# ajaayc/Probability-of-Collision-for-Safe-Planning

Hardware: AMD Instinct MI355X
Metric: particle-waypoint evals/s (GMM+collision) (higher is better)
Workload: dtype f64

## Files before the change

### probability-of-collision-for-safe-planning_amd/csrc/pocs_ctx.hpp

```cpp
#pragma once
#include <hip/hip_runtime.h>

#include <math.h>
#include <stdarg.h>
#include <stdio.h>
#include <stdlib.h>
#include <string.h>

#include <algorithm>
#include <string>
#include <vector>

#include "../../include/pocs.h"
#include "pocs_kernels.h"

#define POCS_HIDDEN __attribute__((visibility("hidden")))

namespace pocs_rt POCS_HIDDEN {

struct DevBuf {
  void* p = nullptr;
  size_t cap = 0;
};

// ... 98 lines not shown
    bool valid = false;
    uint64_t seed = 0, run_index = 0;
    int R = 0;
    unsigned long long epoch = 0;
    std::vector<double> image, chain0, mu0, cov0;
    std::vector<int> slot_plan;
  } ahead;

  pocs_rt::DevBuf d_env, d_sensor, d_hdr, d_chain, d_state, d_param, d_moments, d_partial;
  pocs_rt::DevBuf d_sx, d_sy, d_st, d_flags, d_px, d_py, d_pt, d_hits, d_total, d_ticket, d_tables;
  pocs_rt::DevBuf d_runplan;
  pocs_rt::DevBuf d_surv;
  pocs_rt::DevBuf d_tparent;
  pocs_rt::DevBuf d_world, d_kept, d_keptidx, d_reach;
  pocs_rt::DevBuf d_obsct;
  void* xchg_own = nullptr;
  void* xchg_peer[POCS_XCHG_MAX_WORLD] = {nullptr, nullptr, nullptr, nullptr, nullptr, nullptr, nullptr, nullptr};
  int xchg_world = 0, xchg_rank = -1;
  bool xchg_connected = false;
  unsigned long long xchg_calls = 0;
  double* ext_moments = nullptr;
  long long ext_moments_len = 0;
  void* h_pin = nullptr;
  size_t h_pin_cap = 0;
  void* h_copy = nullptr;
  bool env_dirty = true, sensor_dirty = true;

  hipGraphExec_t graph_gmm = nullptr, graph_mc = nullptr;
  const void* graph_baked[3] = {nullptr, nullptr, nullptr};
  std::string graph_gmm_key, graph_mc_key;

  std::vector<hipEvent_t> events;
  double prof_ms = 0.0;
  long long prof_launches = 0;

  pocs_rt::Results res;
  int last_gmm_adv = -1;
  bool gmm_open = false;
};

namespace pocs_rt POCS_HIDDEN {

inline int fail(pocs_ctx* c, int code, const char* fmt, ...) {
  char buf[512];
  va_list ap;
  va_start(ap, fmt);
  vsnprintf(buf, sizeof buf, fmt, ap);
  va_end(ap);
  if (c) c->err = buf;
  return code;
}

#define HIPCHK(c, call)                                                                   \
  do {                                                                                    \
    hipError_t e_ = (call);                                                               \
    if (e_ != hipSuccess)                                                                 \
      return fail((c), POCS_E_DEVICE, "%s failed: %s (%s:%d)", #call, hipGetErrorString(e_), \
                  __FILE__, __LINE__);                                                    \
  } while (0)

inline void drop_graphs(pocs_ctx* c) {
  if (c->graph_gmm) { hipGraphExecDestroy(c->graph_gmm); c->graph_gmm = nullptr; }
  if (c->graph_mc) { hipGraphExecDestroy(c->graph_mc); c->graph_mc = nullptr; }
  c->graph_gmm_key.clear();
  c->graph_mc_key.clear();
}

inline int ensure(pocs_ctx* c, DevBuf& b, size_t bytes) {
  if (bytes == 0) bytes = 16;
  if (b.cap >= bytes) return POCS_OK;
  if (b.p) {
    HIPCHK(c, hipStreamSynchronize(c->stream));
    drop_graphs(c);
    HIPCHK(c, hipFree(b.p)); b.p = nullptr; b.cap = 0;
  }
  HIPCHK(c, hipMalloc(&b.p, bytes));
  b.cap = bytes;
  return POCS_OK;
}

inline void ra_drop(pocs_ctx* c) {
  if (c->ra_have > 0) c->run_index = c->res.batch_base + (uint64_t)c->res.view + 1;
  c->ra_have = 0;
}
inline void touch(pocs_ctx* c) { ra_drop(c); c->epoch++; }

inline void reset_results(pocs_ctx* c) {
  Results& r = c->res;
// ... 4 lines not shown
  r.plan_slot[0].clear(); r.plan_slot[1].clear(); r.plan_E.clear();
  r.mc_wp.clear(); r.mc_wp_W = 0; r.plan_E_mc.clear();
  r.tree_last = 0; r.tree_sel = 0; r.tree_mc_half = 0;
  r.tree_probs.clear(); r.tree_eval.clear(); r.tree_F.clear(); r.tree_C.clear();
  r.oc_kind = 0; r.oc_M = 0; r.oc_W = 0;
}

inline int world_boxes(const pocs_ctx* c) { return (int)(c->boxes.size() / 5 / (size_t)c->world_S); }
inline const pocs_env_dev* world_at(const pocs_ctx* c, int w) {
  return (const pocs_env_dev*)c->d_env.p + (w < 0 ? 0 : w < c->world_S ? w : c->world_S - 1);
}

static_assert(POCS_MAX_WORLD_RECORDS == POCS_MAX_WORLD_BOXES, "pocs_kernels.h restates the public limit");
inline bool large_world(const pocs_ctx* c) { return !c->world.empty(); }
inline int large_boxes(const pocs_ctx* c) { return (int)(c->world.size() / 5); }

inline double* moments_dev(pocs_ctx* c) { return c->ext_moments ? c->ext_moments : (double*)c->d_moments.p; }
inline long long sample_stride_of(long long count) { return count > 0 ? ((count + 1) & ~1LL) : 2; }
inline uint64_t seed_of_run(const pocs_ctx* c, uint64_t run) { return c->seed + 0x9E3779B97F4A7C15ull * run; }

struct PlanView { const double* traj; const double* odom; int W; };
PlanView plan_view(const pocs_ctx* c, int p);
void compute_chain(pocs_ctx* c, uint64_t seed, const PlanView& pv);
struct PinLayout { size_t chain, state0, runplan, moments, total, end; };
PinLayout pin_layout(const pocs_ctx* c);
int ensure_pin(pocs_ctx* c);
std::vector<int> plan_layout(const pocs_ctx* c, int G);
std::vector<int> slot_lengths(const pocs_ctx* c, const std::vector<int>& slot_plan);
int live_runs(const std::vector<int>& Ws, int lo, int hi, int w);
uint64_t plan_run(const pocs_ctx* c, int p);
void prefetch_next_batch(pocs_ctx* c, int groups);
int stage_and_upload_runs(pocs_ctx* c, int groups, int kind);

int upload_tables(pocs_ctx* c);
int upload_world(pocs_ctx* c);
void fill_gmm_world(const pocs_ctx* c, pocs_gmm_launch* a, int w);
size_t obs_count_words(const pocs_ctx* c);
size_t sync_xwait_offset(const pocs_ctx* c);
void gmm_select_view(pocs_ctx* c, int v);
void tree_select_gmm(pocs_ctx* c, int n);
int run_gmm_full(pocs_ctx* c, double* probability);
int run_mc_local(pocs_ctx* c);

}
```

### probability-of-collision-for-safe-planning_amd/csrc/pocs_host.hip

```cpp
#include <chrono>

#include "pocs_ctx.hpp"

namespace pocs_rt POCS_HIDDEN {

int grid_blocks(long long count, int block, int bpc) {
  long long nb = (count + block - 1) / block;
  if (nb < 1) nb = 1;
  if (nb > 256LL * bpc) nb = 256LL * bpc;
  if (nb > POCS_MAX_BLOCKS) nb = POCS_MAX_BLOCKS;
  return (int)nb;
}
#define POCS_FULL_GRID_FROM_RUNS 4
struct GmmGeometry { long long chunks; int vs_shift; int upb; int blocks; };
GmmGeometry gmm_geometry(long long count, int runs, int K, int groups = 1) {
  const int tb = POCS_GMM_BLOCK_OF(K);
  const long long npairs = (count + 1) / 2;
  GmmGeometry g;
  g.chunks = (npairs + tb - 1) / tb;
  if (g.chunks < 1) g.chunks = 1;
  g.vs_shift = 0;
  while ((2LL << g.vs_shift) <= g.chunks && (2 << g.vs_shift) <= POCS_GMM_MAX_VS) ++g.vs_shift;
  if (runs < 1) runs = 1;
  const long long units = (long long)runs << g.vs_shift;
// ... 112 lines not shown

size_t obs_count_words(const pocs_ctx* c) { return (size_t)c->batch * (size_t)(c->W > 0 ? c->W : 1) * POCS_MAX_OBSTACLES; }
int ensure_obs_counts(pocs_ctx* c) {
  return c->opt_obs_counts ? ensure(c, c->d_obsct, obs_count_words(c) * sizeof(unsigned long long)) : POCS_OK;
}
int enqueue_obs_counts_reset(pocs_ctx* c) {
  if (!c->opt_obs_counts) return POCS_OK;
  HIPCHK(c, pocs_launch_zero_counts((unsigned long long*)c->d_obsct.p, obs_count_words(c), c->stream));
  return POCS_OK;
}
void note_obs_counts(pocs_ctx* c, int kind) {
  c->res.oc_kind = c->opt_obs_counts ? kind : 0;
  c->res.oc_M = world_boxes(c);
  c->res.oc_W = c->W > 0 ? c->W : 1;
}

size_t sync_stop_offset(const pocs_ctx*) { return 4; }
size_t sync_ticket_offset(const pocs_ctx* c) { return 4 + (risk_active(c) ? (((size_t)c->batch + 3) & ~(size_t)3) : 0); }
size_t sync_xwait_offset(const pocs_ctx* c) { return sync_ticket_offset(c) + (size_t)c->batch * (size_t)(c->W > 0 ? c->W : 1); }
size_t sync_words(const pocs_ctx* c) {
  const size_t n = sync_xwait_offset(c) + (size_t)c->batch * (size_t)(c->W > 0 ? c->W : 1);
  return (n + 3) & ~(size_t)3;
}

int gmm_prepare(pocs_ctx* c) {
  if (int r = check_common(c)) return r;
  if (c->K < 1) return fail(c, POCS_E_STATE, "setNumGaussians missing");
  if (c->num_gmm < 1) return fail(c, POCS_E_STATE, "setNumGMMSamples missing");
  long long first, count;
  if (int r = gmm_shard(c, &first, &count)) return r;
  if (int r = upload_static(c)) return r;
  const size_t W = (size_t)c->W, K = (size_t)c->K, R = (size_t)c->batch;
  const GmmGeometry geo = gmm_geometry(count, c->batch, c->K);
  if (int r = ensure(c, c->d_hdr, R * sizeof(pocs_run_header))) return r;
  if (int r = ensure(c, c->d_chain, R * (W > 1 ? W - 1 : 1) * POCS_CHAIN_STRIDE * sizeof(double))) return r;
  if (int r = ensure(c, c->d_state, R * W * K * POCS_STATE_STRIDE * sizeof(double))) return r;
  if (int r = ensure(c, c->d_param, R * W * K * POCS_PARAM_STRIDE * sizeof(double))) return r;
  if (!c->ext_moments)
    if (int r = ensure(c, c->d_moments, W * R * K * POCS_NMOM * sizeof(double))) return r;
  if (c->ext_moments && c->ext_moments_len < (long long)(W * R * K * POCS_NMOM))
    return fail(c, POCS_E_BUFFER, "bound moments buffer too small");
  if (int r = ensure(c, c->d_partial, 2 * ((c->tree.n && R > 256 ? (size_t)256 : R) << geo.vs_shift) * K * POCS_NMOM * sizeof(double))) return r;
  if (int r = ensure(c, c->d_ticket, sync_words(c) * sizeof(unsigned))) return r;
  if (c->plans.n)
    if (int r = ensure(c, c->d_runplan, R * 4 * sizeof(double))) return r;
  if (risk_active(c))
    if (int r = ensure(c, c->d_surv, R * sizeof(double))) return r;
  if (c->tree.n)
    if (int r = upload_tree(c)) return r;
  if (int r = ensure_obs_counts(c)) return r;
  if (large_world(c)) {
    if (int r = ensure(c, c->d_kept, R * POCS_MAX_OBSTACLES * POCS_OBS_STRIDE * sizeof(double))) return r;
    if (int r = ensure(c, c->d_keptidx, R * POCS_MAX_OBSTACLES * sizeof(int))) return r;
    if (int r = ensure(c, c->d_reach, R * W * sizeof(int))) return r;
  }
  if (c->opt_store && !c->tree.n) {
    const size_t n = R * (size_t)sample_stride_of(count);
    if (int r = ensure(c, c->d_sx, n * sizeof(double))) return r;
    if (int r = ensure(c, c->d_sy, n * sizeof(double))) return r;
    if (int r = ensure(c, c->d_st, n * sizeof(double))) return r;
    if (int r = ensure(c, c->d_flags, n * sizeof(int16_t))) return r;
  }
  return ensure_pin(c);
}

int gmm_groups(const pocs_ctx* c) {
  if (c->ext_moments) return 1;
  if (c->tree.n) return 1;
  int g = (int)c->opt_groups;
  if (g == 0) {
    const double count = (double)(c->shard_first >= 0 ? c->shard_count : c->num_gmm);
    g = (c->batch >= 8 && (double)c->batch * count >= 1.2e6) ? 2 : 1;
  }
  if (g > c->batch) g = c->batch;
  return g < 1 ? 1 : g;
}

int gmm_upload_run(pocs_ctx* c) {
  if (int r = stage_and_upload_runs(c, gmm_groups(c), 0)) return r;
  const PinLayout pl = pin_layout(c);
  double* pin = (double*)c->h_pin;
  const int W = c->W, R = c->batch;
  const size_t row = (size_t)c->K * POCS_STATE_STRIDE * sizeof(double);
  HIPCHK(c, hipMemcpy2DAsync(c->d_state.p, (size_t)W * row, pin + pl.state0, row, row, (size_t)(c->tree.n ? 1 : R),
                             hipMemcpyHostToDevice, c->stream));
  return POCS_OK;
}

bool whole_call_exchanges(const pocs_ctx* c) { return c->xchg_connected && c->shard_first >= 0 && !c->ext_moments; }

void fill_gmm_world(const pocs_ctx* c, pocs_gmm_launch* a, int w) {
  a->env = world_at(c, w);
  a->tables = (const pocs_tables*)c->d_tables.p;
  a->fp = c->fp; a->M = world_boxes(c);
  a->fp_rr = sqrt(c->fp.hx * c->fp.hx + c->fp.hy * c->fp.hy); a->fp_phi = atan2(c->fp.hy, c->fp.hx);
  if (large_world(c)) {
    a->world = (const double*)c->d_world.p; a->world_M = large_boxes(c);
    a->kept = (double*)c->d_kept.p; a->kept_idx = (int*)c->d_keptidx.p; a->reach = (int*)c->d_reach.p;
  }
}

void fill_gmm_launch(pocs_ctx* c, pocs_gmm_launch* a, long long first, long long count, int w,
// ... 125 lines not shown
          continue;
        }
      }
      if (int r = enqueue_step(c, first, count, w, true, exchange, (prof && g == 0) ? w : -1, st, lo, cnt, G, lone, adv, risk)) return r;
    }
  if (lone) {
    pocs_gmm_launch a;
    fill_gmm_launch(c, &a, first, count, W - 1, 0, 1, 1);
    set_lone(c, &a, W - 1);
    HIPCHK(c, pocs_launch_gmm_close(c->K, a, c->stream));
  }
  for (int g = 1; g < G; ++g) {
    HIPCHK(c, hipEventRecord(c->ev_join[g - 1], c->side_stream[g - 1]));
    HIPCHK(c, hipStreamWaitEvent(c->stream, c->ev_join[g - 1], 0));
  }
  if (prof) HIPCHK(c, hipEventRecord(c->ev_seq[1], c->stream));
  return POCS_OK;
}
int enqueue_gmm_results(pocs_ctx* c) {
  const int W = c->W;
  const PinLayout pl = pin_layout(c);
  HIPCHK(c, hipMemcpyAsync((double*)c->h_pin + pl.moments, moments_dev(c),
                           (size_t)W * c->batch * c->K * POCS_NMOM * sizeof(double), hipMemcpyDeviceToHost, c->stream));
  static_assert(POCS_SYNC_ABORT == 1, "the stop words follow the give-up word and two pad words");
  HIPCHK(c, hipMemcpyAsync((double*)c->h_pin + pl.total + c->batch + 1, (unsigned*)c->d_ticket.p + POCS_SYNC_ABORT,
                           (risk_active(c) ? 3 + (size_t)c->batch : 1) * sizeof(unsigned), hipMemcpyDeviceToHost, c->stream));
  if (large_world(c)) {
    c->reach.assign((size_t)c->batch * (size_t)c->W, 0);
    HIPCHK(c, hipMemcpyAsync(c->reach.data(), c->d_reach.p, c->reach.size() * sizeof(int), hipMemcpyDeviceToHost, c->stream));
  }
  return POCS_OK;
}

int gmm_read_reach(pocs_ctx* c) {
  const int R = c->batch, W = c->W;
  const bool plans = c->plans.n && !c->res.plan_slot[0].empty();
  const std::vector<int> by_slot = c->reach;
  c->reach_R = R; c->reach_W = W;
  c->reach_len.assign((size_t)R, W);
  int bad_w = -1, bad_n = 0, bad_r = 0;
  for (int r = 0; r < R; ++r) {
    const int slot = plans ? c->res.plan_slot[0][(size_t)r] : r;
    if (plans) c->reach_len[(size_t)r] = c->plans.W[(size_t)r];
    for (int w = 0; w < W; ++w) {
      const int n = by_slot[(size_t)slot * W + w];
      c->reach[(size_t)r * W + w] = n;
      if (n > POCS_MAX_OBSTACLES && (bad_w < 0 || w < bad_w)) { bad_w = w; bad_n = n; bad_r = r; }
    }
  }
  if (bad_w >= 0)
    return fail(c, POCS_E_STATE, "large world: %d boxes are in reach of run %d at waypoint %d, more than the %d a run may meet at one waypoint; results discarded",
                bad_n, bad_r, bad_w, POCS_MAX_OBSTACLES);
  return POCS_OK;
}

double waypoint_probability(const double* row, int K, long long n) {
  double coll = 0.0;
  for (int k = 0; k < K; ++k) coll += row[(size_t)k * POCS_NMOM + 1];
  return coll / (1.0 * (double)n);
}
// ... 137 lines not shown
  HIPCHK(c, e);
  e = hipGraphInstantiate(&exec, g, nullptr, nullptr, 0);
  hipGraphDestroy(g);
  HIPCHK(c, e);
  have = key;
  return POCS_OK;
}

int run_gmm_full(pocs_ctx* c, double* probability) {
  if (!probability) return fail(c, POCS_E_ARG, "null output");
#if defined(POCS_TUNING) && defined(POCS_CALL_TIMES)
  const auto t_in = std::chrono::steady_clock::now();
  auto lap = [&](const char* what) { fprintf(stderr, "[call] %s +%.1f us\n", what,
      std::chrono::duration<double, std::micro>(std::chrono::steady_clock::now() - t_in).count()); };
#else
  auto lap = [](const char*) {};
#endif
  c->res.oc_kind = 0;
  c->reach.clear(); c->reach_len.clear(); c->reach_R = 0; c->reach_W = 0;
  if (int r = gmm_prepare(c)) return r;
  long long first, count;
  if (int r = gmm_shard(c, &first, &count)) return r;
  lap("prepared");
  if (whole_call_exchanges(c)) {
    if (c->batch > POCS_XCHG_MAX_RUNS) return fail(c, POCS_E_ARG, "exchange: at most %d runs per call", POCS_XCHG_MAX_RUNS);
    c->xchg_calls += 1;
  }
  if (int r = gmm_upload_run(c)) return r;
  lap("upload enqueued");
  const bool prof = c->opt_profile == 1 && !c->tree.n, span = c->opt_profile == 2 && c->opt_graph;
  if (int r = prof_begin(c, gmm_hot_launches(c))) return r;
#if defined(POCS_TUNING) && defined(POCS_GRAPH_WITH_COPIES)
  const bool copies_in_graph = c->opt_graph && !prof;
#else
  const bool copies_in_graph = false;
#endif
  if (!copies_in_graph) if (int r = enqueue_ticket_reset(c)) return r;
  if (c->opt_graph && c->opt_profile != 1) {
    if (int r = ensure_graph(c, c->graph_gmm, c->graph_gmm_key, config_key(c, first, count, "gmm"), [&] {
          int r = copies_in_graph ? enqueue_ticket_reset(c) : POCS_OK;
          if (!r) r = enqueue_gmm_all(c, first, count, false);
          if (!r && copies_in_graph) r = enqueue_gmm_results(c);
          if (copies_in_graph) {
            c->graph_baked[0] = c->d_ticket.p; c->graph_baked[1] = c->h_pin; c->graph_baked[2] = moments_dev(c);
          }
          return r;
        })) return r;
    if (copies_in_graph && (c->graph_baked[0] != c->d_ticket.p || c->graph_baked[1] != c->h_pin || c->graph_baked[2] != moments_dev(c)))
      return fail(c, POCS_E_STATE, "a pointer baked into the graph's memset / memcpy nodes changed between capture and replay");
    if (span) HIPCHK(c, hipEventRecord(c->ev_seq[0], c->stream));
    HIPCHK(c, hipGraphLaunch(c->graph_gmm, c->stream));
    if (span) HIPCHK(c, hipEventRecord(c->ev_seq[1], c->stream));
  } else {
    if (int r = enqueue_gmm_all(c, first, count, prof)) return r;
  }
  if (!copies_in_graph) if (int r = enqueue_gmm_results(c)) return r;
  lap("launched");
  prefetch_next_batch(c, gmm_groups(c));
  lap("next batch prepared");
  HIPCHK(c, hipStreamSynchronize(c->stream));
  lap("synchronised");
  if (prof) if (int r = prof_collect(c, gmm_hot_launches(c))) return r;
  if (prof || span) {
    float ms = 0.f;
    HIPCHK(c, hipEventElapsedTime(&ms, c->ev_seq[0], c->ev_seq[1]));
    c->seq_ms = ms; c->seq_groups = gmm_groups(c);
    if (span) { c->prof_ms = ms; c->prof_launches = (long long)gmm_hot_launches(c); }
  }
  {
    const PinLayout pl = pin_layout(c);
    unsigned gave_up = 0;
    memcpy(&gave_up, (double*)c->h_pin + pl.total + c->batch + 1, sizeof gave_up);
    if (gave_up) return fail(c, POCS_E_DEVICE, "a bounded wait expired on the device (code %u); results discarded", gave_up);
    const unsigned* stop = risk_active(c) ? (const unsigned*)((double*)c->h_pin + pl.total + c->batch + 1) + 3 : nullptr;
    if (large_world(c)) if (int r = gmm_read_reach(c)) { reset_results(c); return r; }
    if (int r = gmm_combine(c, (double*)c->h_pin + pl.moments, probability, stop)) { reset_results(c); return r; }
  }
  note_obs_counts(c, 1);
  c->res.last_gmm_count = count;
  c->res.last_gmm_wp = c->W - 1;
  lap("combined");
  return POCS_OK;
}

int mc_shard(pocs_ctx* c, long long* first, long long* count) {
  *first = c->shard_first >= 0 ? c->shard_first : 0;
  *count = c->shard_first >= 0 ? c->shard_count : c->num_particles;
  if (*first < 0 || *count < 0 || *first + *count > c->num_particles)
    return fail(c, POCS_E_ARG, "shard [%lld,+%lld) outside numParticles=%lld", *first, *count, c->num_particles);
  return POCS_OK;
}

bool mc_stop_active(const pocs_ctx* c) { return c->opt_mc_rb && risk_active(c) && !c->tree.n; }
bool mc_counts_active(const pocs_ctx* c) { return c->opt_mc_wp || c->opt_obs_counts || mc_stop_active(c); }
bool mc_fused_form(const pocs_ctx* c) { return c->opt_fused && !mc_stop_active(c); }
size_t mc_total_words(const pocs_ctx* c) {
  const size_t R = (size_t)c->batch, W = (size_t)c->W;
// ... 367 lines not shown
  a.xchg.world = c->xchg_world; a.xchg.rank = c->xchg_rank;
  a.xchg.epoch = (c->xchg_calls << 20) | (unsigned long long)(w + 1);
  a.xchg.parity = (int)((c->xchg_calls * (unsigned long long)c->W + (unsigned long long)w) & 1ull);
  const int slot = c->opt_profile == 1 ? w : -1;
  if (slot >= 0) HIPCHK(c, hipEventRecord(c->events[2 * slot], c->stream));
  HIPCHK(c, pocs_launch_gmm_step(c->K, a, c->stream));
  if (slot >= 0) HIPCHK(c, hipEventRecord(c->events[2 * slot + 1], c->stream));
  c->res.last_gmm_wp = w;
  c->res.last_gmm_count = count;
  if (w + 1 < c->W) c->last_gmm_adv = w + 1;
  return POCS_OK;
}

int pocs_gmm_end(pocs_ctx* c, double* probability) {
  if (!c) return POCS_E_ARG;
  if (!c->gmm_open) return fail(c, POCS_E_ORDER, "pocs_gmm_end before pocs_gmm_begin");
  if (c->res.last_gmm_wp != c->W - 1) return fail(c, POCS_E_ORDER, "pocs_gmm_end after %d of %d waypoints", c->res.last_gmm_wp + 1, c->W);
  if (!probability) return fail(c, POCS_E_ARG, "null output");
  const PinLayout pl = pin_layout(c);
  if (int r = enqueue_gmm_results(c)) return r;
  prefetch_next_batch(c, gmm_groups(c));
  HIPCHK(c, hipStreamSynchronize(c->stream));
  unsigned gave_up = 0;
  memcpy(&gave_up, (double*)c->h_pin + pl.total + c->batch + 1, sizeof gave_up);
  if (gave_up) { c->gmm_open = false; return fail(c, POCS_E_DEVICE, "a bounded wait expired on the device (code %u: 4 = a peer's moments never arrived); results discarded", gave_up); }
  if (int r = prof_collect(c, (size_t)c->W)) return r;
  (void)gmm_combine(c, (double*)c->h_pin + pl.moments, probability);
  note_obs_counts(c, 1);
  c->gmm_open = false;
  return POCS_OK;
}

}
```

### probability-of-collision-for-safe-planning_amd/csrc/pocs_kernels.h

```cpp
#pragma once
#include <hip/hip_runtime.h>
#include <stdint.h>
#include "pocs_collide.h"
#include "pocs_model.h"
#include "pocs_world.h"

#define POCS_BLOCK 256
#define POCS_GMM_BLOCK_OF(K) 512
#define POCS_GMM_BLOCKS_PER_CU 2
#define POCS_NUM_CUS 256
#define POCS_MAX_BLOCKS 2048
#define POCS_GMM_MAX_VS 256
static_assert(POCS_GMM_BLOCK_OF(3) == 512 && POCS_GMM_MAX_VS == 256, "summation tree (numerics v7 and later): 512-pair chunks, 256 virtual slices");
#define POCS_LONE_PRE 3
#define POCS_GMM_SUB 32
#define POCS_UNIT_SUMS 10
#define POCS_FLUSH_ROWS 5
#define POCS_FLUSH_PITCH 66
#define POCS_CHAIN_Z 10
#define POCS_CHAIN_STRIDE 48
static_assert(POCS_CHAIN_Z + POCS_MAX_LANDMARKS <= POCS_CHAIN_STRIDE, "chain record too small");

struct pocs_env_dev {
  pocs_footprint fp;
// ... 91 lines not shown
  double mu0[3];
  double L0[6];
  const double* run_plan;
  int step;
  int nruns;
  int nontemporal;
  int wp_mode;
  unsigned long long* wp_counts;
  unsigned* wp_stop;
  long long wp_n;
  double wp_bound;
  const int* tree_parent;
  const double* tree_sx; const double* tree_sy; const double* tree_sth;
  const uint32_t* tree_shits;
  int tree_lo, tree_dst_lo, tree_src_lo, tree_pad;
  int env_steps;
  int env_pad;
  unsigned long long* obs_counts;
  const double* world;
  int world_M;
  int world_pad;
};


hipError_t pocs_launch_gmm_step(int K, const pocs_gmm_launch& a, hipStream_t s);
hipError_t pocs_launch_world_cull(int K, const pocs_gmm_launch& a, hipStream_t s);
hipError_t pocs_launch_gmm_advance(int K, const pocs_gmm_launch& a, hipStream_t s);
hipError_t pocs_launch_gmm_tree_advance(int K, const pocs_gmm_launch& a, hipStream_t s);
hipError_t pocs_launch_gmm_tree_step(int K, const pocs_gmm_launch& a, hipStream_t s);
hipError_t pocs_launch_gmm_close(int K, const pocs_gmm_launch& a, hipStream_t s);
hipError_t pocs_launch_gmm_exchange(int K, const pocs_gmm_launch& a, const pocs_xchg_dev& x, hipStream_t s);
hipError_t pocs_launch_zero_counts(unsigned long long* p, size_t words, hipStream_t s);
hipError_t pocs_launch_copy(const void* src, void* dst, long long bytes, hipStream_t s);
hipError_t pocs_launch_fill(void* dst, long long bytes, hipStream_t s);
hipError_t pocs_launch_probe_math(const pocs_tables* tables, int n, const uint32_t* wr, const uint32_t* wa, const double* x, double* out, hipStream_t s);
hipError_t pocs_launch_probe_collide(int K, const pocs_gmm_launch& a, int n, const double* x, const double* y, const double* th,
                                     int* flags, int* nkeep, double* kept, hipStream_t s);
hipError_t pocs_launch_mc_init(int nblk, const pocs_mc_launch& a, hipStream_t s);
hipError_t pocs_launch_mc_step(int nblk, const pocs_mc_launch& a, hipStream_t s);
hipError_t pocs_launch_mc_fused(int nblk, const pocs_mc_launch& a, hipStream_t s);
hipError_t pocs_launch_mc_count(int nblk, const pocs_mc_launch& a, hipStream_t s);
hipError_t pocs_launch_mc_tree_step(int nblk, const pocs_mc_launch& a, hipStream_t s);
```

### probability-of-collision-for-safe-planning_amd/csrc/pocs_kernels.hip

```cpp
#include "pocs_kernels.h"
#include <type_traits>
#include <stdio.h>

namespace {
#include "pocs_dev_prims.hpp"
#include "pocs_dev_advance.hpp"
#include "pocs_dev_gmm.hpp"
#include "pocs_dev_mc.hpp"

template <typename F>
hipError_t with_K(const int K, F f) {
  static_assert(POCS_MAX_GAUSSIANS == 8, "one case per K");
  switch (K) {
    case 1: return f(std::integral_constant<int, 1>());
    case 2: return f(std::integral_constant<int, 2>());
    case 3: return f(std::integral_constant<int, 3>());
    case 4: return f(std::integral_constant<int, 4>());
    case 5: return f(std::integral_constant<int, 5>());
    case 6: return f(std::integral_constant<int, 6>());
    case 7: return f(std::integral_constant<int, 7>());
    case 8: return f(std::integral_constant<int, 8>());
    default: return hipErrorInvalidValue;
  }
}
// ... 165 lines not shown
    if (a.env_steps > 1) hipLaunchKernelGGL(k_mc_fused_sched<MC_COUNTS | MC_BOXES>, dim3(nblk, a.nruns), dim3(POCS_BLOCK), 0, s, a);
    else                 hipLaunchKernelGGL(k_mc_fused_boxes, dim3(nblk, a.nruns), dim3(POCS_BLOCK), 0, s, a);
  } else if (a.env_steps > 1) {
    if (a.wp_mode) hipLaunchKernelGGL(k_mc_fused_sched<MC_COUNTS>, dim3(nblk, a.nruns), dim3(POCS_BLOCK), 0, s, a);
    else           hipLaunchKernelGGL(k_mc_fused_sched<MC_PLAIN>, dim3(nblk, a.nruns), dim3(POCS_BLOCK), 0, s, a);
  } else if (a.wp_mode) hipLaunchKernelGGL(k_mc_fused_counts, dim3(nblk, a.nruns), dim3(POCS_BLOCK), 0, s, a);
  else                  hipLaunchKernelGGL(k_mc_fused, dim3(nblk, a.nruns), dim3(POCS_BLOCK), 0, s, a);
  return hipGetLastError();
}
hipError_t pocs_launch_mc_count(int nblk, const pocs_mc_launch& a, hipStream_t s) {
  hipLaunchKernelGGL(k_mc_count, dim3(nblk, a.nruns), dim3(POCS_BLOCK), 0, s, a);
  return hipGetLastError();
}

__global__ __launch_bounds__(POCS_BLOCK) void k_zero_counts(unsigned long long* __restrict__ p, size_t n) {
  const size_t stride = (size_t)gridDim.x * POCS_BLOCK;
  for (size_t i = (size_t)blockIdx.x * POCS_BLOCK + threadIdx.x; i < n; i += stride) p[i] = 0ull;
}
hipError_t pocs_launch_zero_counts(unsigned long long* p, size_t words, hipStream_t s) {
  if (!p) return hipErrorInvalidValue;
  if (words == 0) return hipSuccess;
  const size_t nb = (words + POCS_BLOCK - 1) / POCS_BLOCK;
  hipLaunchKernelGGL(k_zero_counts, dim3((unsigned)(nb < POCS_MAX_BLOCKS ? nb : POCS_MAX_BLOCKS)), dim3(POCS_BLOCK), 0, s, p, words);
  return hipGetLastError();
}

__global__ __launch_bounds__(POCS_BLOCK) void k_copy(const double2* __restrict__ src, double2* __restrict__ dst, long long n) {
  typedef double v2d __attribute__((ext_vector_type(2)));
  const v2d* s = reinterpret_cast<const v2d*>(src);
  v2d* d = reinterpret_cast<v2d*>(dst);
  const long long stride = (long long)gridDim.x * POCS_BLOCK * 4;
  for (long long i = (long long)blockIdx.x * POCS_BLOCK * 4 + threadIdx.x; i < n; i += stride) {
    v2d v[4];
#pragma unroll
    for (int u = 0; u < 4; ++u) if (i + u * POCS_BLOCK < n) v[u] = __builtin_nontemporal_load(s + i + u * POCS_BLOCK);
#pragma unroll
    for (int u = 0; u < 4; ++u) if (i + u * POCS_BLOCK < n) __builtin_nontemporal_store(v[u], d + i + u * POCS_BLOCK);
  }
}
__global__ __launch_bounds__(POCS_BLOCK) void k_fill(double2* __restrict__ dst, long long n, double v) {
  typedef double v2d __attribute__((ext_vector_type(2)));
  v2d* d = reinterpret_cast<v2d*>(dst);
  const v2d x = {v, v};
  const long long stride = (long long)gridDim.x * POCS_BLOCK * 4;
  for (long long i = (long long)blockIdx.x * POCS_BLOCK * 4 + threadIdx.x; i < n; i += stride) {
#pragma unroll
// ... 81 lines not shown
```

### probability-of-collision-for-safe-planning_amd/csrc/pocs_stage.hip

```cpp
#include "pocs_ctx.hpp"

namespace pocs_rt POCS_HIDDEN {

void inverse_odometry(const double p1[3], const double p2[3], double out[3]) {
  double r1 = atan2(p2[1] - p1[1], p2[0] - p1[0]) - p1[2];
  r1 = pocs_wrap_angle(r1);
  const double ddx = p2[0] - p1[0], ddy = p2[1] - p1[1];
  const double tr = sqrt(ddx * ddx + ddy * ddy);
  double r2 = p2[2] - p1[2] - r1;
  r2 = pocs_wrap_angle(r2);
  out[0] = r1; out[1] = tr; out[2] = r2;
}

double chain_normal(uint64_t seed, int step, int draw) {
  const pocs_u32x4 w = pocs_draw(seed, (uint64_t)step, 0u, POCS_STREAM_CHAIN, (uint32_t)(draw >> 1));
  double n0, n1;
  pocs_normal_pair(w.x, w.y, w.z, &n0, &n1);
  return (draw & 1) ? n1 : n0;
}

PlanView plan_view(const pocs_ctx* c, int p) {
  if (p < 0) return PlanView{c->traj.data(), c->odom.data(), c->W};
  return PlanView{c->plans.traj.data() + c->plans.toff[(size_t)p], c->plans.odom.data() + c->plans.ooff[(size_t)p], c->plans.W[(size_t)p]};
}
// ... 50 lines not shown
  memcpy(cov, c->cov0, sizeof cov);
  double real[3] = {mu[0], mu[1], mu[2]};
  for (int i = 0; i < W - 1; ++i) {
    double* rec = &c->res.h_chain[(size_t)i * POCS_CHAIN_STRIDE];
    const double us[3] = {odom[i], odom[(W - 1) + i], odom[2 * (W - 1) + i]};
    const double xs[3] = {traj[i], traj[W + i], traj[2 * W + i]};
    const double xg[3] = {traj[i + 1], traj[W + i + 1], traj[2 * W + i + 1]};
    chain_step(c, seed, i, us, xs, xg, mu, cov, real, rec);
    memcpy(&c->res.h_mu[(size_t)i * 3], mu, sizeof mu);
    memcpy(&c->res.h_cov[(size_t)i * 9], cov, sizeof cov);
  }
}

PinLayout pin_layout(const pocs_ctx* c) {
  PinLayout p;
  const size_t W = (size_t)(c->W > 0 ? c->W : 1), K = (size_t)(c->K > 0 ? c->K : 1), R = (size_t)c->batch;
  p.chain = 2 * R;
  p.state0 = p.chain + R * (W > 1 ? W - 1 : 1) * POCS_CHAIN_STRIDE;
  p.runplan = p.state0 + R * K * POCS_STATE_STRIDE;
  p.moments = p.runplan + (c->plans.n ? 4 * R : 0);
  p.total = p.moments + W * R * K * POCS_NMOM;
  p.end = p.total + R + 2 + (R + 4) / 2 + 1;
  if (c->opt_mc_wp || c->opt_mc_rb || c->opt_obs_counts) p.end += R * W + (R + 1) / 2;
  if (c->tree.n) p.end += R;
  return p;
}

int ensure_pin(pocs_ctx* c) {
  const size_t bytes = pin_layout(c).end * sizeof(double);
  if (c->h_pin_cap >= bytes) return POCS_OK;
  if (c->h_pin) { HIPCHK(c, hipHostFree(c->h_pin)); c->h_pin = nullptr; c->h_pin_cap = 0; }
  HIPCHK(c, hipHostMalloc(&c->h_pin, bytes, hipHostMallocDefault));
  c->h_pin_cap = bytes;
  drop_graphs(c);
  return POCS_OK;
}

uint64_t effective_seed(const pocs_ctx* c, uint64_t ahead = 0) {
  return seed_of_run(c, c->run_index + ahead);
}

std::vector<int> plan_layout(const pocs_ctx* c, int G) {
  std::vector<int> slot_plan;
  if (!c->plans.n) return slot_plan;
  const int R = c->plans.n;
  if (G < 1) G = 1;
  if (G > R) G = R;
  std::vector<int> rank(R);
  for (int p = 0; p < R; ++p) rank[p] = p;
  std::stable_sort(rank.begin(), rank.end(), [c](int x, int y) { return c->plans.W[(size_t)x] > c->plans.W[(size_t)y]; });
  std::vector<int> lo(G), n(G), fill(G, 0), order(G);
  for (int g = 0; g < G; ++g) {
    lo[g] = (int)((long long)g * R / G);
    n[g] = (int)((long long)(g + 1) * R / G) - lo[g];
    order[g] = g;
// ... 77 lines not shown
    const double start[3] = {pv.traj[0], pv.traj[pv.W], pv.traj[2 * pv.W]};
    write_initial_mixture(img + pl.state0 + (size_t)r * (c->K > 0 ? c->K : 0) * POCS_STATE_STRIDE, start, c->cov0, c->K);
    if (c->plans.n) {
      double* q = img + pl.runplan + 4 * (size_t)r;
      q[0] = start[0]; q[1] = start[1]; q[2] = start[2]; q[3] = (double)(pv.W - 1);
    }
  }
}

void prefetch_next_batch(pocs_ctx* c, int groups) {
  const PinLayout pl = pin_layout(c);
  auto& a = c->ahead;
  if (c->tree.n) { a.valid = false; return; }
  std::vector<double> keep_chain = c->res.h_chain, keep_mu = c->res.h_mu, keep_cov = c->res.h_cov;
  a.image.resize(pl.moments);
  a.slot_plan = plan_layout(c, groups);
  build_run_image(c, 0, a.image.data(), a.slot_plan);
  a.chain0.swap(c->res.h_chain); a.mu0.swap(c->res.h_mu); a.cov0.swap(c->res.h_cov);
  c->res.h_chain.swap(keep_chain); c->res.h_mu.swap(keep_mu); c->res.h_cov.swap(keep_cov);
  a.seed = c->seed; a.run_index = c->run_index; a.R = c->batch; a.epoch = c->epoch;
  a.valid = true;
}

int stage_and_upload_runs(pocs_ctx* c, int groups, int kind) {
  const PinLayout pl = pin_layout(c);
  double* pin = (double*)c->h_pin;
  const int W = c->W, R = c->batch;
  const size_t steps = (size_t)(W > 1 ? W - 1 : 1);
  const std::vector<int> slot_plan = plan_layout(c, groups);
  auto& a = c->ahead;
  if (a.valid && a.seed == c->seed && a.run_index == c->run_index && a.R == R && a.epoch == c->epoch &&
      a.image.size() == pl.moments && a.slot_plan == slot_plan) {
    memcpy(pin, a.image.data(), pl.moments * sizeof(double));
    c->res.h_chain = a.chain0; c->res.h_mu = a.mu0; c->res.h_cov = a.cov0;
  } else {
    build_run_image(c, 0, pin, slot_plan);
  }
  a.valid = false;
  for (int r = 0; r < R; ++r) ((uint64_t*)pin)[2 * (size_t)r + 1] = c->xchg_calls;
  c->res.batch_base = c->run_index;
  c->res.batch_R = R;
  c->res.view = 0;
  c->run_index += (c->plans.n && c->opt_plan_seeds) || c->tree.n ? 1 : (uint64_t)R;
  if (c->plans.n) {
    std::vector<int>& ps = c->res.plan_slot[kind];
    ps.assign((size_t)R, 0);
    for (int r = 0; r < R; ++r) ps[(size_t)slot_plan[(size_t)r]] = r;
    HIPCHK(c, hipMemcpyAsync(c->d_runplan.p, pin + pl.runplan, (size_t)R * 4 * sizeof(double), hipMemcpyHostToDevice, c->stream));
  }
  HIPCHK(c, hipMemcpyAsync(c->d_hdr.p, pin, (size_t)R * sizeof(pocs_run_header), hipMemcpyHostToDevice, c->stream));
  HIPCHK(c, hipMemcpyAsync(c->d_chain.p, pin + pl.chain, (size_t)R * steps * POCS_CHAIN_STRIDE * sizeof(double),
                           hipMemcpyHostToDevice, c->stream));
  return POCS_OK;
}

}
```

Before: 171.7 billion.

## Replace per-call memcpys with mapped-pinned intake/outtake kernels inside the graph

Allocates the pinned staging block as host-mapped memory and adds gather kernels that read inputs from and write results to it directly. These kernels replace the several hipMemcpyAsync and memset calls around each GMM call and are captured into the hipGraph. A stamp check skips rebuilding the graph when the configuration has not changed. The aim is to cut per-call API and DMA-setup overhead. In exchange, copies now cross PCIe/fabric from inside a kernel (zero-copy access), which can be slower for large moment buffers.

```diff
diff --git a/probability-of-collision-for-safe-planning_amd/csrc/pocs_ctx.hpp b/probability-of-collision-for-safe-planning_amd/csrc/pocs_ctx.hpp
--- a/probability-of-collision-for-safe-planning_amd/csrc/pocs_ctx.hpp
+++ b/probability-of-collision-for-safe-planning_amd/csrc/pocs_ctx.hpp
@@ -144,13 +144,15 @@
   double* ext_moments = nullptr;
   long long ext_moments_len = 0;
   void* h_pin = nullptr;
+  void* h_pin_dev = nullptr;
   size_t h_pin_cap = 0;
   void* h_copy = nullptr;
   bool env_dirty = true, sensor_dirty = true;
 
   hipGraphExec_t graph_gmm = nullptr, graph_mc = nullptr;
-  const void* graph_baked[3] = {nullptr, nullptr, nullptr};
+  const void* graph_baked = nullptr;
   std::string graph_gmm_key, graph_mc_key;
+  struct { unsigned long long epoch = 0; long long first = -1, count = -1; int xworld = 0; bool valid = false; } graph_gmm_stamp;
 
   std::vector<hipEvent_t> events;
   double prof_ms = 0.0;
@@ -186,6 +188,7 @@
   if (c->graph_mc) { hipGraphExecDestroy(c->graph_mc); c->graph_mc = nullptr; }
   c->graph_gmm_key.clear();
   c->graph_mc_key.clear();
+  c->graph_gmm_stamp.valid = false;
 }
 
 inline int ensure(pocs_ctx* c, DevBuf& b, size_t bytes) {
@@ -236,7 +239,7 @@
 struct PlanView { const double* traj; const double* odom; int W; };
 PlanView plan_view(const pocs_ctx* c, int p);
 void compute_chain(pocs_ctx* c, uint64_t seed, const PlanView& pv);
-struct PinLayout { size_t chain, state0, runplan, moments, total, end; };
+struct PinLayout { size_t chain, state0, runplan, moments, total, reach, end; };
 PinLayout pin_layout(const pocs_ctx* c);
 int ensure_pin(pocs_ctx* c);
 std::vector<int> plan_layout(const pocs_ctx* c, int G);
@@ -244,7 +247,7 @@
 int live_runs(const std::vector<int>& Ws, int lo, int hi, int w);
 uint64_t plan_run(const pocs_ctx* c, int p);
 void prefetch_next_batch(pocs_ctx* c, int groups);
-int stage_and_upload_runs(pocs_ctx* c, int groups, int kind);
+int stage_and_upload_runs(pocs_ctx* c, int groups, int kind, bool upload = true);
 
 int upload_tables(pocs_ctx* c);
 int upload_world(pocs_ctx* c);
diff --git a/probability-of-collision-for-safe-planning_amd/csrc/pocs_host.hip b/probability-of-collision-for-safe-planning_amd/csrc/pocs_host.hip
--- a/probability-of-collision-for-safe-planning_amd/csrc/pocs_host.hip
+++ b/probability-of-collision-for-safe-planning_amd/csrc/pocs_host.hip
@@ -158,6 +158,10 @@
   const size_t n = sync_xwait_offset(c) + (size_t)c->batch * (size_t)(c->W > 0 ? c->W : 1);
   return (n + 3) & ~(size_t)3;
 }
+
+static_assert(POCS_SYNC_ABORT == 1, "the give-up word lies in front of the stop words");
+size_t sync_result_words(const pocs_ctx* c) { return risk_active(c) ? sync_stop_offset(c) + (size_t)c->batch : 2; }
+unsigned* pin_sync_words(const pocs_ctx* c, const PinLayout& pl) { return (unsigned*)((double*)c->h_pin + pl.total + c->batch + 1); }
 
 int gmm_prepare(pocs_ctx* c) {
   if (int r = check_common(c)) return r;
@@ -188,7 +192,7 @@
   if (large_world(c)) {
     if (int r = ensure(c, c->d_kept, R * POCS_MAX_OBSTACLES * POCS_OBS_STRIDE * sizeof(double))) return r;
     if (int r = ensure(c, c->d_keptidx, R * POCS_MAX_OBSTACLES * sizeof(int))) return r;
-    if (int r = ensure(c, c->d_reach, R * W * sizeof(int))) return r;
+    if (int r = ensure(c, c->d_reach, ((R * W + 1) & ~(size_t)1) * sizeof(int))) return r;
   }
   if (c->opt_store && !c->tree.n) {
     const size_t n = R * (size_t)sample_stride_of(count);
@@ -212,8 +216,9 @@
   return g < 1 ? 1 : g;
 }
 
-int gmm_upload_run(pocs_ctx* c) {
-  if (int r = stage_and_upload_runs(c, gmm_groups(c), 0)) return r;
+int gmm_upload_run(pocs_ctx* c, bool upload = true) {
+  if (int r = stage_and_upload_runs(c, gmm_groups(c), 0, upload)) return r;
+  if (!upload) return POCS_OK;
   const PinLayout pl = pin_layout(c);
   double* pin = (double*)c->h_pin;
   const int W = c->W, R = c->batch;
@@ -385,20 +390,54 @@
   const PinLayout pl = pin_layout(c);
   HIPCHK(c, hipMemcpyAsync((double*)c->h_pin + pl.moments, moments_dev(c),
                            (size_t)W * c->batch * c->K * POCS_NMOM * sizeof(double), hipMemcpyDeviceToHost, c->stream));
-  static_assert(POCS_SYNC_ABORT == 1, "the stop words follow the give-up word and two pad words");
-  HIPCHK(c, hipMemcpyAsync((double*)c->h_pin + pl.total + c->batch + 1, (unsigned*)c->d_ticket.p + POCS_SYNC_ABORT,
-                           (risk_active(c) ? 3 + (size_t)c->batch : 1) * sizeof(unsigned), hipMemcpyDeviceToHost, c->stream));
-  if (large_world(c)) {
-    c->reach.assign((size_t)c->batch * (size_t)c->W, 0);
-    HIPCHK(c, hipMemcpyAsync(c->reach.data(), c->d_reach.p, c->reach.size() * sizeof(int), hipMemcpyDeviceToHost, c->stream));
-  }
+  HIPCHK(c, hipMemcpyAsync(pin_sync_words(c, pl), c->d_ticket.p, sync_result_words(c) * sizeof(unsigned), hipMemcpyDeviceToHost, c->stream));
+  if (large_world(c))
+    HIPCHK(c, hipMemcpyAsync((double*)c->h_pin + pl.reach, c->d_reach.p, (size_t)c->batch * (size_t)c->W * sizeof(int), hipMemcpyDeviceToHost, c->stream));
+  return POCS_OK;
+}
+
+void call_part(pocs_call_io* io, const void* src, void* dst, size_t rows, size_t row_words, size_t src_pitch, size_t dst_pitch) {
+  if (!rows || !row_words) return;
+  pocs_call_part& q = io->part[io->parts++];
+  q.src = (const unsigned long long*)src; q.dst = (unsigned long long*)dst;
+  q.rows = rows; q.row_words = row_words; q.src_pitch = src_pitch; q.dst_pitch = dst_pitch;
+}
+int enqueue_call_intake(pocs_ctx* c) {
+  const PinLayout pl = pin_layout(c);
+  const double* pin = (const double*)c->h_pin_dev;
+  const size_t W = (size_t)c->W, K = (size_t)c->K, R = (size_t)c->batch, steps = W > 1 ? W - 1 : 1;
+  pocs_call_io io;
+  memset(&io, 0, sizeof io);
+  static_assert(sizeof(pocs_run_header) == 16, "a run header is two words of the pinned block");
+  call_part(&io, pin, c->d_hdr.p, 1, 2 * R, 2 * R, 2 * R);
+  call_part(&io, pin + pl.chain, c->d_chain.p, 1, R * steps * POCS_CHAIN_STRIDE, R * steps * POCS_CHAIN_STRIDE, R * steps * POCS_CHAIN_STRIDE);
+  if (c->plans.n) call_part(&io, pin + pl.runplan, c->d_runplan.p, 1, 4 * R, 4 * R, 4 * R);
+  call_part(&io, pin + pl.state0, c->d_state.p, c->tree.n ? 1 : R, K * POCS_STATE_STRIDE, K * POCS_STATE_STRIDE, W * K * POCS_STATE_STRIDE);
+  call_part(&io, nullptr, c->d_ticket.p, 1, sync_words(c) / 2, 0, sync_words(c) / 2);
+  if (large_world(c)) call_part(&io, nullptr, c->d_reach.p, 1, (R * W + 1) / 2, 0, (R * W + 1) / 2);
+  HIPCHK(c, pocs_launch_call_intake(io, c->stream));
+  return POCS_OK;
+}
+int enqueue_call_outtake(pocs_ctx* c) {
+  const PinLayout pl = pin_layout(c);
+  double* pin = (double*)c->h_pin_dev;
+  const size_t W = (size_t)c->W, K = (size_t)c->K, R = (size_t)c->batch, nm = W * R * K * POCS_NMOM;
+  pocs_call_io io;
+  memset(&io, 0, sizeof io);
+  call_part(&io, c->d_moments.p, pin + pl.moments, 1, nm, nm, nm);
+  const size_t sw = (sync_result_words(c) + 1) / 2;
+  call_part(&io, c->d_ticket.p, pin + pl.total + R + 1, 1, sw, sw, sw);
+  if (large_world(c)) call_part(&io, c->d_reach.p, pin + pl.reach, 1, (R * W + 1) / 2, (R * W + 1) / 2, (R * W + 1) / 2);
+  HIPCHK(c, pocs_launch_call_outtake(io, c->stream));
   return POCS_OK;
 }
 
 int gmm_read_reach(pocs_ctx* c) {
   const int R = c->batch, W = c->W;
   const bool plans = c->plans.n && !c->res.plan_slot[0].empty();
-  const std::vector<int> by_slot = c->reach;
+  const int* pinned = (const int*)((double*)c->h_pin + pin_layout(c).reach);
+  const std::vector<int> by_slot(pinned, pinned + (size_t)R * (size_t)W);
+  c->reach.assign(by_slot.size(), 0);
   c->reach_R = R; c->reach_W = W;
   c->reach_len.assign((size_t)R, W);
   int bad_w = -1, bad_n = 0, bad_r = 0;
@@ -582,39 +621,43 @@
   long long first, count;
   if (int r = gmm_shard(c, &first, &count)) return r;
   lap("prepared");
-  if (whole_call_exchanges(c)) {
-    if (c->batch > POCS_XCHG_MAX_RUNS) return fail(c, POCS_E_ARG, "exchange: at most %d runs per call", POCS_XCHG_MAX_RUNS);
-    c->xchg_calls += 1;
-  }
-  if (int r = gmm_upload_run(c)) return r;
-  lap("upload enqueued");
+  const bool exchanges = whole_call_exchanges(c);
+  if (exchanges && c->batch > POCS_XCHG_MAX_RUNS) return fail(c, POCS_E_ARG, "exchange: at most %d runs per call", POCS_XCHG_MAX_RUNS);
   const bool prof = c->opt_profile == 1 && !c->tree.n, span = c->opt_profile == 2 && c->opt_graph;
-  if (int r = prof_begin(c, gmm_hot_launches(c))) return r;
-#if defined(POCS_TUNING) && defined(POCS_GRAPH_WITH_COPIES)
-  const bool copies_in_graph = c->opt_graph && !prof;
-#else
-  const bool copies_in_graph = false;
-#endif
-  if (!copies_in_graph) if (int r = enqueue_ticket_reset(c)) return r;
-  if (c->opt_graph && c->opt_profile != 1) {
-    if (int r = ensure_graph(c, c->graph_gmm, c->graph_gmm_key, config_key(c, first, count, "gmm"), [&] {
-          int r = copies_in_graph ? enqueue_ticket_reset(c) : POCS_OK;
-          if (!r) r = enqueue_gmm_all(c, first, count, false);
-          if (!r && copies_in_graph) r = enqueue_gmm_results(c);
-          if (copies_in_graph) {
-            c->graph_baked[0] = c->d_ticket.p; c->graph_baked[1] = c->h_pin; c->graph_baked[2] = moments_dev(c);
-          }
-          return r;
-        })) return r;
-    if (copies_in_graph && (c->graph_baked[0] != c->d_ticket.p || c->graph_baked[1] != c->h_pin || c->graph_baked[2] != moments_dev(c)))
-      return fail(c, POCS_E_STATE, "a pointer baked into the graph's memset / memcpy nodes changed between capture and replay");
-    if (span) HIPCHK(c, hipEventRecord(c->ev_seq[0], c->stream));
-    HIPCHK(c, hipGraphLaunch(c->graph_gmm, c->stream));
-    if (span) HIPCHK(c, hipEventRecord(c->ev_seq[1], c->stream));
-  } else {
-    if (int r = enqueue_gmm_all(c, first, count, prof)) return r;
-  }
-  if (!copies_in_graph) if (int r = enqueue_gmm_results(c)) return r;
+  if (exchanges) c->xchg_calls += 1;
+  auto enqueue_call = [&]() -> int {
+    if (int r = gmm_upload_run(c, false)) return r;
+    lap("staged");
+    if (int r = prof_begin(c, gmm_hot_launches(c))) return r;
+    auto launches = [&](bool timed) -> int {
+      if (int r = enqueue_call_intake(c)) return r;
+      if (int r = enqueue_gmm_all(c, first, count, timed)) return r;
+      return c->ext_moments ? POCS_OK : enqueue_call_outtake(c);
+    };
+    if (c->opt_graph && c->opt_profile != 1) {
+      auto& st = c->graph_gmm_stamp;
+      const int xworld = exchanges ? c->xchg_world : 0;
+      if (!(c->graph_gmm && st.valid && st.epoch == c->epoch && st.first == first && st.count == count && st.xworld == xworld)) {
+        if (int r = ensure_graph(c, c->graph_gmm, c->graph_gmm_key, config_key(c, first, count, "gmm"), [&] {
+              c->graph_baked = c->h_pin_dev;
+              return launches(false);
+            })) return r;
+        st.epoch = c->epoch; st.first = first; st.count = count; st.xworld = xworld; st.valid = true;
+      }
+      if (c->graph_baked != c->h_pin_dev)
+        return fail(c, POCS_E_STATE, "the pinned block's address baked into the graph's first and last launch changed between capture and replay");
+      if (span) HIPCHK(c, hipEventRecord(c->ev_seq[0], c->stream));
+      HIPCHK(c, hipGraphLaunch(c->graph_gmm, c->stream));
+      if (span) HIPCHK(c, hipEventRecord(c->ev_seq[1], c->stream));
+    } else {
+      if (int r = launches(prof)) return r;
+    }
+    return c->ext_moments ? enqueue_gmm_results(c) : POCS_OK;
+  };
+  if (int r = enqueue_call()) {
+    if (exchanges) c->xchg_calls -= 1;
+    return r;
+  }
   lap("launched");
   prefetch_next_batch(c, gmm_groups(c));
   lap("next batch prepared");
@@ -630,9 +673,9 @@
   {
     const PinLayout pl = pin_layout(c);
     unsigned gave_up = 0;
-    memcpy(&gave_up, (double*)c->h_pin + pl.total + c->batch + 1, sizeof gave_up);
+    memcpy(&gave_up, pin_sync_words(c, pl) + POCS_SYNC_ABORT, sizeof gave_up);
     if (gave_up) return fail(c, POCS_E_DEVICE, "a bounded wait expired on the device (code %u); results discarded", gave_up);
-    const unsigned* stop = risk_active(c) ? (const unsigned*)((double*)c->h_pin + pl.total + c->batch + 1) + 3 : nullptr;
+    const unsigned* stop = risk_active(c) ? pin_sync_words(c, pl) + sync_stop_offset(c) : nullptr;
     if (large_world(c)) if (int r = gmm_read_reach(c)) { reset_results(c); return r; }
     if (int r = gmm_combine(c, (double*)c->h_pin + pl.moments, probability, stop)) { reset_results(c); return r; }
   }
@@ -1046,7 +1089,7 @@
   prefetch_next_batch(c, gmm_groups(c));
   HIPCHK(c, hipStreamSynchronize(c->stream));
   unsigned gave_up = 0;
-  memcpy(&gave_up, (double*)c->h_pin + pl.total + c->batch + 1, sizeof gave_up);
+  memcpy(&gave_up, pin_sync_words(c, pl) + POCS_SYNC_ABORT, sizeof gave_up);
   if (gave_up) { c->gmm_open = false; return fail(c, POCS_E_DEVICE, "a bounded wait expired on the device (code %u: 4 = a peer's moments never arrived); results discarded", gave_up); }
   if (int r = prof_collect(c, (size_t)c->W)) return r;
   (void)gmm_combine(c, (double*)c->h_pin + pl.moments, probability);
diff --git a/probability-of-collision-for-safe-planning_amd/csrc/pocs_kernels.h b/probability-of-collision-for-safe-planning_amd/csrc/pocs_kernels.h
--- a/probability-of-collision-for-safe-planning_amd/csrc/pocs_kernels.h
+++ b/probability-of-collision-for-safe-planning_amd/csrc/pocs_kernels.h
@@ -137,6 +137,19 @@
   int world_pad;
 };
 
+#define POCS_CALL_IO_PARTS 6
+struct pocs_call_part {
+  const unsigned long long* src;
+  unsigned long long* dst;
+  unsigned long long rows, row_words, src_pitch, dst_pitch;
+};
+struct pocs_call_io {
+  pocs_call_part part[POCS_CALL_IO_PARTS];
+  int parts;
+  int pad;
+};
+hipError_t pocs_launch_call_intake(const pocs_call_io& io, hipStream_t s);
+hipError_t pocs_launch_call_outtake(const pocs_call_io& io, hipStream_t s);
 
 hipError_t pocs_launch_gmm_step(int K, const pocs_gmm_launch& a, hipStream_t s);
 hipError_t pocs_launch_world_cull(int K, const pocs_gmm_launch& a, hipStream_t s);
diff --git a/probability-of-collision-for-safe-planning_amd/csrc/pocs_kernels.hip b/probability-of-collision-for-safe-planning_amd/csrc/pocs_kernels.hip
--- a/probability-of-collision-for-safe-planning_amd/csrc/pocs_kernels.hip
+++ b/probability-of-collision-for-safe-planning_amd/csrc/pocs_kernels.hip
@@ -211,6 +211,45 @@
   if (words == 0) return hipSuccess;
   const size_t nb = (words + POCS_BLOCK - 1) / POCS_BLOCK;
   hipLaunchKernelGGL(k_zero_counts, dim3((unsigned)(nb < POCS_MAX_BLOCKS ? nb : POCS_MAX_BLOCKS)), dim3(POCS_BLOCK), 0, s, p, words);
+  return hipGetLastError();
+}
+
+__device__ __forceinline__ void call_io_block(const pocs_call_io& io) {
+  const unsigned long long stride = (unsigned long long)gridDim.x * POCS_BLOCK;
+  for (int p = 0; p < io.parts; ++p) {
+    const pocs_call_part q = io.part[p];
+    const unsigned long long n = q.rows * q.row_words;
+    for (unsigned long long i = (unsigned long long)blockIdx.x * POCS_BLOCK + threadIdx.x; i < n; i += stride) {
+      const unsigned long long row = i / q.row_words, col = i - row * q.row_words;
+      q.dst[row * q.dst_pitch + col] = q.src ? q.src[row * q.src_pitch + col] : 0ull;
+    }
+  }
+}
+__global__ __launch_bounds__(POCS_BLOCK) void k_call_intake(pocs_call_io io) { call_io_block(io); }
+__global__ __launch_bounds__(POCS_BLOCK) void k_call_outtake(pocs_call_io io) { call_io_block(io); }
+static hipError_t call_io_grid(const pocs_call_io& io, unsigned* blocks) {
+  if (io.parts < 0 || io.parts > POCS_CALL_IO_PARTS) return hipErrorInvalidValue;
+  unsigned long long most = 1;
+  for (int p = 0; p < io.parts; ++p) {
+    const pocs_call_part& q = io.part[p];
+    if (!q.dst || (((uintptr_t)q.dst | (uintptr_t)q.src) & 7u) || q.row_words < 1 || q.dst_pitch < q.row_words || (q.src && q.src_pitch < q.row_words))
+      return hipErrorInvalidValue;
+    if (q.rows * q.row_words > most) most = q.rows * q.row_words;
+  }
+  const unsigned long long nb = (most + POCS_BLOCK - 1) / POCS_BLOCK;
+  *blocks = (unsigned)(nb < POCS_NUM_CUS ? nb : POCS_NUM_CUS);
+  return hipSuccess;
+}
+hipError_t pocs_launch_call_intake(const pocs_call_io& io, hipStream_t s) {
+  unsigned nb = 1;
+  if (hipError_t e = call_io_grid(io, &nb)) return e;
+  hipLaunchKernelGGL(k_call_intake, dim3(nb), dim3(POCS_BLOCK), 0, s, io);
+  return hipGetLastError();
+}
+hipError_t pocs_launch_call_outtake(const pocs_call_io& io, hipStream_t s) {
+  unsigned nb = 1;
+  if (hipError_t e = call_io_grid(io, &nb)) return e;
+  hipLaunchKernelGGL(k_call_outtake, dim3(nb), dim3(POCS_BLOCK), 0, s, io);
   return hipGetLastError();
 }
 
diff --git a/probability-of-collision-for-safe-planning_amd/csrc/pocs_stage.hip b/probability-of-collision-for-safe-planning_amd/csrc/pocs_stage.hip
--- a/probability-of-collision-for-safe-planning_amd/csrc/pocs_stage.hip
+++ b/probability-of-collision-for-safe-planning_amd/csrc/pocs_stage.hip
@@ -96,6 +96,8 @@
   p.total = p.moments + W * R * K * POCS_NMOM;
   p.end = p.total + R + 2 + (R + 4) / 2 + 1;
   if (c->opt_mc_wp || c->opt_mc_rb || c->opt_obs_counts) p.end += R * W + (R + 1) / 2;
+  p.reach = p.end;
+  if (large_world(c)) p.end += (R * W + 1) / 2;
   if (c->tree.n) p.end += R;
   return p;
 }
@@ -103,8 +105,12 @@
 int ensure_pin(pocs_ctx* c) {
   const size_t bytes = pin_layout(c).end * sizeof(double);
   if (c->h_pin_cap >= bytes) return POCS_OK;
-  if (c->h_pin) { HIPCHK(c, hipHostFree(c->h_pin)); c->h_pin = nullptr; c->h_pin_cap = 0; }
-  HIPCHK(c, hipHostMalloc(&c->h_pin, bytes, hipHostMallocDefault));
+  if (c->h_pin) {
+    HIPCHK(c, hipStreamSynchronize(c->stream));
+    HIPCHK(c, hipHostFree(c->h_pin)); c->h_pin = nullptr; c->h_pin_dev = nullptr; c->h_pin_cap = 0;
+  }
+  HIPCHK(c, hipHostMalloc(&c->h_pin, bytes, hipHostMallocMapped));
+  HIPCHK(c, hipHostGetDevicePointer(&c->h_pin_dev, c->h_pin, 0));
   c->h_pin_cap = bytes;
   drop_graphs(c);
   return POCS_OK;
@@ -228,7 +234,7 @@
   a.valid = true;
 }
 
-int stage_and_upload_runs(pocs_ctx* c, int groups, int kind) {
+int stage_and_upload_runs(pocs_ctx* c, int groups, int kind, bool upload) {
   const PinLayout pl = pin_layout(c);
   double* pin = (double*)c->h_pin;
   const int W = c->W, R = c->batch;
@@ -252,8 +258,9 @@
     std::vector<int>& ps = c->res.plan_slot[kind];
     ps.assign((size_t)R, 0);
     for (int r = 0; r < R; ++r) ps[(size_t)slot_plan[(size_t)r]] = r;
-    HIPCHK(c, hipMemcpyAsync(c->d_runplan.p, pin + pl.runplan, (size_t)R * 4 * sizeof(double), hipMemcpyHostToDevice, c->stream));
-  }
+    if (upload) HIPCHK(c, hipMemcpyAsync(c->d_runplan.p, pin + pl.runplan, (size_t)R * 4 * sizeof(double), hipMemcpyHostToDevice, c->stream));
+  }
+  if (!upload) return POCS_OK;
   HIPCHK(c, hipMemcpyAsync(c->d_hdr.p, pin, (size_t)R * sizeof(pocs_run_header), hipMemcpyHostToDevice, c->stream));
   HIPCHK(c, hipMemcpyAsync(c->d_chain.p, pin + pl.chain, (size_t)R * steps * POCS_CHAIN_STRIDE * sizeof(double),
                            hipMemcpyHostToDevice, c->stream));
```

After: 172.6 billion, median of 6. No clear change (+0.5%).
